# dusk-network/plonk

Measured on AMD Instinct MI355X. Metric: prove() wall-clock (ms) at 2^20 gates, lower is better.
Workload: dtype u32 limbs (Fr 256-bit / Fp 384-bit Montgomery)

## Files before the change

### __graft_entry__.py

```python
from __future__ import annotations

import concurrent.futures as cf
import os
import shutil
import subprocess
import sys

ROOT = os.path.dirname(os.path.abspath(__file__))
CSRC = os.path.join(ROOT, "plonk_amd", "csrc")
LIBDIR = os.path.join(ROOT, "plonk_amd", "lib")
OBJDIR = os.path.join(ROOT, "build", "obj")
LIB = os.path.join(LIBDIR, "libplonk_hip.so")
HIP_SOURCES = ["ntt.hip", "msm.hip", "msm_sort.hip", "capi.hip", "poly.hip", "prover.hip", "serial.hip", "comm.hip", "verify.hip", "diagnose.hip", "kzg.hip", "composer.hip", "msm_points.hip"]
MSM_LARGE_BITS = os.environ.get("PLONK_BUILD_MSM_LARGE_BITS", "19")
MSM_MEDIUM = os.environ.get("PLONK_BUILD_MSM_MEDIUM", "") == "1"
HIP_VARIANTS = [("msm.hip", "nbl" + MSM_LARGE_BITS, ["-DPLONK_MSM_NB_BITS=" + MSM_LARGE_BITS]),
                ("msm_sort.hip", "nbl" + MSM_LARGE_BITS, ["-DPLONK_MSM_NB_BITS=" + MSM_LARGE_BITS])]
if MSM_MEDIUM:
    HIP_VARIANTS += [("msm.hip", "nbm17", ["-DPLONK_MSM_NB_BITS=17", "-DPLONK_MSM_WITH_MEDIUM"]),
                     ("msm_sort.hip", "nbm17", ["-DPLONK_MSM_NB_BITS=17", "-DPLONK_MSM_WITH_MEDIUM"])]
    HIP_FLAGS_EXTRA = ["-DPLONK_MSM_WITH_MEDIUM"]
else:
    HIP_FLAGS_EXTRA = []
HIPCC = shutil.which("hipcc") or "/opt/rocm/bin/hipcc"
# ... 59 lines not shown
def build_dev_arith(verbose: bool = True) -> str:
    src = os.path.join(ROOT, "tests", "csrc", "dev_arith.hip")
    if not os.path.exists(src):
        return DEV_ARITH_LIB
    deps = [src, os.path.join(ROOT, "tests", "csrc", "arith_cases.hpp")] + _headers()
    if _newer(DEV_ARITH_LIB, deps):
        os.makedirs(os.path.dirname(DEV_ARITH_LIB), exist_ok=True)
        os.makedirs(OBJDIR, exist_ok=True)

        def compile_group(group: str) -> str:
            obj = os.path.join(OBJDIR, "dev_arith." + group + ".o")
            if _newer(obj, deps):
                subprocess.check_call([HIPCC, *HIP_FLAGS, "-DARITH_GROUP=ARITH_FAMILIES_" + group, "-c", src, "-o", obj])
            return obj

        with cf.ThreadPoolExecutor(max_workers=len(DEV_ARITH_GROUPS)) as ex:
            objs = list(ex.map(compile_group, DEV_ARITH_GROUPS))
        subprocess.check_call([HIPCC, "--offload-arch=gfx950", "-shared", "-fPIC", *objs, "-o", DEV_ARITH_LIB])
    if verbose:
        print(f"[build] {DEV_ARITH_LIB}")
    return DEV_ARITH_LIB


def build() -> None:
    with cf.ThreadPoolExecutor(max_workers=1) as side:
        dev_arith = side.submit(build_dev_arith)
        build_hip()
        build_oracle()
        build_fake_rccl()
        dev_arith.result()
    sys.path.insert(0, ROOT)
    import plonk_amd
    plonk_amd.load_library()


def smoke() -> None:
    sys.path.insert(0, ROOT)
    import random

    import plonk_amd
    from oracle import bls12_381 as E
    from oracle.fft import EvaluationDomain

    ctx = plonk_amd.Context(0)
    rnd = random.Random(7)
    L = 12
    coeffs = [rnd.randrange(E.Q) for _ in range((1 << 9) + 3)]
    got = ctx.ntt(coeffs, L, inverse=False, coset=True)
    assert got == EvaluationDomain(1 << L).coset_fft(coeffs), "NTT mismatch vs oracle"
    pts = [E.g1_mul(E.G1_GEN, rnd.randrange(1, E.Q)) for _ in range(64)]
# ... 9 lines not shown
```

### plonk_amd/csrc/poly.hip

```cpp
#include <cstdlib>

#include "plonk_internal.hpp"
#include "fr29.cuh"
#include "fp_safegcd.cuh"
#include "poly.hpp"

namespace plonk {

__device__ __forceinline__ Fr ldf(const Fr* p) {
  const uint4* q = reinterpret_cast<const uint4*>(p);
  uint4 a = q[0], b = q[1];
  Fr r;
  r.l[0] = a.x; r.l[1] = a.y; r.l[2] = a.z; r.l[3] = a.w;
  r.l[4] = b.x; r.l[5] = b.y; r.l[6] = b.z; r.l[7] = b.w;
  return r;
}
__device__ __forceinline__ void stf(Fr* p, const Fr& v) {
  uint4* q = reinterpret_cast<uint4*>(p);
  q[0] = make_uint4(v.l[0], v.l[1], v.l[2], v.l[3]);
  q[1] = make_uint4(v.l[4], v.l[5], v.l[6], v.l[7]);
}
__device__ __forceinline__ Fr small(uint32_t v, const Fr& one) {
  Fr acc = Fr::zero();
  Fr p = one;
  for (uint32_t b = v; b; b >>= 1) {
    if (b & 1) acc = acc + p;
    p = p.dbl();
  }
  return acc;
}

__global__ void fill_zero_kernel(Fr* p, uint64_t n) {
  const uint64_t i = (uint64_t)blockIdx.x * blockDim.x + threadIdx.x;
  if (i < n) stf(p + i, Fr::zero());
}

__global__ void blind_kernel(Fr* coeffs, uint64_t n, BlindArgs a) {
  const int i = threadIdx.x;
  if (i < a.count) {
    const Fr low = (uint64_t)i >= n ? a.b[i - n] : ldf(coeffs + i);
    stf(coeffs + i, low - a.b[i]);
    if (n + i >= (uint64_t)a.count) stf(coeffs + n + i, a.b[i]);
  }
}

__global__ void split_t_kernel(Fr* __restrict__ t, uint64_t n, uint64_t np, Fr* __restrict__ out, SplitArgs a) {
  const uint64_t i = (uint64_t)blockIdx.x * blockDim.x + threadIdx.x;
  const int part = blockIdx.y;
  if (i >= np) return;
  Fr v = Fr::zero();
  if (i < n) v = ldf(t + (uint64_t)part * n + i);
  else if (i == n) v = a.b[part];
  if (part >= 1 && i == 0) v = v - a.b[part - 1];
  stf(out + (uint64_t)part * np + i, v);
  if (part == 0 && i == n + 1) stf(t + 3 * n, ldf(t + 3 * n) - a.b[2]);
}

__global__ void __launch_bounds__(256) trimmed_len_kernel(const Fr* __restrict__ p, uint64_t n, unsigned long long* out) {
  __shared__ unsigned long long sh[256];
  const uint64_t i = (uint64_t)blockIdx.x * blockDim.x + threadIdx.x;
  unsigned long long v = 0;
  if (i < n && !ldf(p + i).is_zero()) v = i + 1;
  sh[threadIdx.x] = v;
  __syncthreads();
  for (int d = 128; d >= 1; d >>= 1) {
    if ((int)threadIdx.x < d) { const unsigned long long o = sh[threadIdx.x + d]; if (o > sh[threadIdx.x]) sh[threadIdx.x] = o; }
// ... 405 lines not shown
  }
  const uint64_t r = i - 1;
  Fr29 root = ld_slot(a.tw_lo29, r & ((1ull << a.lobits) - 1));
  if (a.use_hi) root = Fr29::mul(root, ld_slot(a.tw_hi29, r >> a.lobits));
  const Fr29 conv = tw29(k.conv), gamma_t = tw29(k.gamma_t), b32 = tw29(k.b32_t);
  Fr29 num, den;
#pragma unroll
  for (int j = 0; j < 4; ++j) {
    const Fr29 wg = Fr29::add_csub(Fr29::mul(ld29_(a.wires[j] + r), conv), gamma_t);
    const Fr29 nf = Fr29::add_csub(wg, Fr29::mul(root, tw29(k.bk_t[j])));
    const Fr29 df = Fr29::add_csub(wg, Fr29::mul(ld29_(a.sigma[j] + r), b32));
    num = j ? Fr29::mul(num, nf) : nf;
    den = j ? Fr29::mul(den, df) : df;
  }
  stf(a.num + i, num.to_fr());
  stf(a.den + i, den.to_fr());
}
__global__ void mul_arrays_kernel(Fr* __restrict__ a, const Fr* __restrict__ b, uint64_t n, int* zero_flag) {
  const uint64_t i = (uint64_t)blockIdx.x * blockDim.x + threadIdx.x;
  if (i >= n) return;
  const Fr y = ldf(b + i);
  if (zero_flag && y.is_zero()) *zero_flag = 1;
  stf(a + i, Fr29::mul(ld29_(a + i), Fr29::from_fr(y)).to_fr());
}

__device__ __forceinline__ Fr delta4(const Fr& f, const Fr& one) {
  const Fr two = one.dbl();
  return f * (f - one) * (f - two) * (f - two - one);
}

__device__ __forceinline__ Fr29 ld29(const Fr* p) { return Fr29::from_fr(ldf(p)); }
__device__ __forceinline__ Fr29 c29(const uint32_t (&v)[9]) {
  Fr29 r;
#pragma unroll
  for (int i = 0; i < 9; ++i) r.l[i] = v[i];
  return r;
}

struct WidgetConst {
  Tw conv, one_r, c1, c3, c9, c18, c81, c83, ed;
  Tw rg[4];
  Tw lg[5];
  Tw fx[4];
  Tw vr[3];
};
template <bool WIDGETS>
// ... 236 lines not shown
  if (first >= n) return;
  const Fr29 add = Fr29::from_fr(a.addend);
  const uint64_t e = first + exp_off;
  Fr29 p = tw29(a.one_t);
  bool started = false;
#pragma unroll 1
  for (uint32_t b = 0; b < a.nbits; ++b) {
    if ((e >> b) & 1) {
      const Fr29 w = tw29(a.pw[b]);
      p = started ? Fr29::mul(p, w) : w;
      started = true;
    }
  }
  const Fr29 step = tw29(a.pw[6]);
#pragma unroll 1
  for (int k = 0; k < E; ++k) {
    const uint64_t i = first + 64ull * k;
    if (i >= n) break;
    stf(dst + i, Fr29::mul(Fr29::add_csub(ld29_(src + i + src_off), add), p).to_fr());
    if (E > 1) p = Fr29::mul(p, step);
  }
}

__global__ void fold_kernel(const Fr* __restrict__ src, Fr* __restrict__ dst, uint64_t n, uint32_t extra, Fr c) {
  const uint64_t i = (uint64_t)blockIdx.x * blockDim.x + threadIdx.x;
  if (i >= n) return;
  Fr v = ldf(src + i);
  if (i < extra) v = v + c * ldf(src + n + i);
  stf(dst + i, v);
}

__global__ void shard_pack_kernel(ShardPackArgs a) {
  const uint64_t i = (uint64_t)blockIdx.x * blockDim.x + threadIdx.x;
  const uint32_t k = blockIdx.y, peer = blockIdx.z;
  if (i >= a.stride) return;
  const Fr* F = a.F[k];
  Fr v = Fr::zero();
  if (i < a.per) {
    const uint64_t idx = (uint64_t)peer * a.per + i;
    if (idx < a.n) v = ldf(F + idx);
  } else {
    v = ldf(F + (i - a.per));
  }
  stf(a.send + ((uint64_t)peer * a.cpr + k) * a.stride + i, v);
}

// ... 31 lines not shown
}

__global__ void shard_split_fix_kernel(ShardSplitFix a) {
  if (threadIdx.x != 0) return;
  auto own = [&](uint64_t idx) { return idx >= a.lo && idx < a.hi; };
  if (own(a.n)) { stf(a.parts[0] + a.n, a.b[0]); stf(a.parts[1] + a.n, a.b[1]); stf(a.parts[2] + a.n, a.b[2]); }
  if (own(0)) {
    stf(a.parts[1], ldf(a.parts[1]) - a.b[0]);
    stf(a.parts[2], ldf(a.parts[2]) - a.b[1]);
    stf(a.parts[3], ldf(a.parts[3]) - a.b[2]);
  }
}

static inline dim3 grid1(uint64_t n, int t) { return dim3((uint32_t)((n + t - 1) / t)); }

int poly_fill_zero(Ctx* c, Fr* p, uint64_t n) {
  if (!n) return PLONK_OK;
  hipLaunchKernelGGL(fill_zero_kernel, grid1(n, 256), dim3(256), 0, c->stream, p, n);
  HIP_TRY(hipGetLastError());
  return PLONK_OK;
}
int poly_blind(Ctx* c, Fr* coeffs, uint64_t n, const BlindArgs& a) {
  hipLaunchKernelGGL(blind_kernel, dim3(1), dim3(64), 0, c->stream, coeffs, n, a);
  HIP_TRY(hipGetLastError());
  return PLONK_OK;
}
int poly_split_t(Ctx* c, Fr* t, uint64_t n, uint64_t np, Fr* out, const SplitArgs& a) {
  hipLaunchKernelGGL(split_t_kernel, dim3((uint32_t)((np + 255) / 256), 3), dim3(256), 0, c->stream, t, n, np, out, a);
  HIP_TRY(hipGetLastError());
  return PLONK_OK;
}
int poly_trimmed_len(Ctx* c, const Fr* p, uint64_t n, unsigned long long* out_dev) {
  HIP_TRY(hipMemsetAsync(out_dev, 0, sizeof(unsigned long long), c->stream));
  hipLaunchKernelGGL(trimmed_len_kernel, grid1(n, 256), dim3(256), 0, c->stream, p, n, out_dev);
  HIP_TRY(hipGetLastError());
  return PLONK_OK;
}
int poly_sigma_evals(Ctx* c, const uint32_t* map_dev, const Fr* roots, Fr* out, uint64_t n, uint64_t stride, const SigmaArgs& a) {
  dim3 grid = grid1(n, 256);
  grid.y = 4;
  hipLaunchKernelGGL(sigma_evals_kernel, grid, dim3(256), 0, c->stream, map_dev, roots, out, n, stride, a);
  HIP_TRY(hipGetLastError());
  return PLONK_OK;
}
int poly_gather_wires(Ctx* c, const uint32_t* idx_dev, const Fr* values, Fr* wires, uint64_t constraints, uint64_t n) {
  dim3 grid = grid1(n, 256);
// ... 27 lines not shown
  else if (cfg == 2) BI_LAUNCH(64, 16);
  else if (cfg == 3) BI_LAUNCH(128, 8);
  else BI_LAUNCH(256, 16);
#undef BI_LAUNCH
  HIP_TRY(hipGetLastError());
  return PLONK_OK;
}
int poly_perm_terms(Ctx* c, const PermArgs& a) {
  PermConst k;
  k.conv = tw_of(Fr::from_u64(32));
  k.gamma_t = tw_of(a.gamma);
  for (int j = 0; j < 4; ++j) k.bk_t[j] = tw_of(a.beta * a.ks[j]);
  k.b32_t = tw_of(a.beta * Fr::from_u64(32));
  k.one_t = tw_of(Fr::one());
  PermArgs r = a;
  if (r.count == 0) { r.first = 0; r.count = a.n; }
  if (r.first + r.count > a.n) return (plonk::set_last_error("invalid argument", __func__, __FILE__, __LINE__), PLONK_ERR_ARG);
  hipLaunchKernelGGL(perm_terms_kernel, grid1(r.count, 128), dim3(128), 0, c->stream, r, k);
  HIP_TRY(hipGetLastError());
  return PLONK_OK;
}
int poly_mul_arrays(Ctx* c, Fr* a, const Fr* b, uint64_t n, int* zero_flag) {
  hipLaunchKernelGGL(mul_arrays_kernel, grid1(n, 256), dim3(256), 0, c->stream, a, b, n, zero_flag);
  HIP_TRY(hipGetLastError());
  return PLONK_OK;
}
int poly_quotient(Ctx* c, const QuotientArgs& q) {
  prof_begin(c, 3);
  WidgetConst wc{};
  if (q.has[QS_RANGE] | q.has[QS_LOGIC] | q.has[QS_FIXED] | q.has[QS_VAR]) {
    wc.conv = tw_of(Fr::from_u64(32));
    wc.one_r = tw_plain(Fr::one());
    wc.c1 = tw_of(Fr::one()); wc.c3 = tw_of(Fr::from_u64(3)); wc.c9 = tw_of(Fr::from_u64(9));
    wc.c18 = tw_of(Fr::from_u64(18)); wc.c81 = tw_of(Fr::from_u64(81)); wc.c83 = tw_of(Fr::from_u64(83));
    wc.ed = tw_of(q.edwards_d);
    Fr k = q.range_ch.sqr(), w = q.range_ch;
    for (int j = 0; j < 4; ++j) { wc.rg[j] = tw_of(w); w = w * k; }
    k = q.logic_ch.sqr();
    const Fr lk[5] = {k.sqr() * k, Fr::one(), k, k.sqr(), k.sqr().sqr()};
    for (int j = 0; j < 5; ++j) wc.lg[j] = tw_of(lk[j] * q.logic_ch);
    k = q.fixed_ch.sqr(); w = q.fixed_ch;
    for (int j = 0; j < 4; ++j) { wc.fx[j] = tw_of(w); w = w * k; }
    k = q.var_ch.sqr(); w = q.var_ch;
    for (int j = 0; j < 3; ++j) { wc.vr[j] = tw_of(w); w = w * k; }
    hipLaunchKernelGGL(quotient_kernel<true>, grid1(q.n8, 128), dim3(128), 0, c->stream, q, wc);
  } else {
// ... 106 lines not shown
  while (nbits < MP_BITS && (emax >> nbits)) ++nbits;
  Fr29 p = Fr29::twiddle_from_fr(x);
  for (uint32_t b = 0; b < nbits; ++b) {
    for (int i = 0; i < 9; ++i) a.pw[b].w[i] = p.l[i];
    p = Fr29::mul(p, p);
  }
  a.one_t = tw_of(Fr::one());
  a.addend = addend;
  a.nbits = nbits;
  a.zero_at = zero_at;
  if (n <= (1ull << 17)) hipLaunchKernelGGL(mul_powers_kernel<1>, grid1(n, 256), dim3(256), 0, c->stream, src, dst, n, a, src_off, exp_off);
  else if (n <= (1ull << 19)) hipLaunchKernelGGL(mul_powers_kernel<4>, grid1((n + 3) / 4 + 64, 256), dim3(256), 0, c->stream, src, dst, n, a, src_off, exp_off);
  else hipLaunchKernelGGL(mul_powers_kernel<16>, grid1((n + 15) / 16 + 64, 256), dim3(256), 0, c->stream, src, dst, n, a, src_off, exp_off);
}
int poly_ruffini(Ctx* c, const Fr* src, Fr* dst, uint64_t len, const Fr& z, const Fr& zinv, Fr* scratch, Fr* totals) {
  launch_mul_powers(c, src, scratch, len, z, 0, 0);
  int rc = scan_suffix_sum(c, scratch, len, totals);
  if (rc) return rc;
  launch_mul_powers(c, scratch, dst, len - 1, zinv, 1, 1, Fr::zero(), len - 1);
  HIP_TRY(hipGetLastError());
  return PLONK_OK;
}

__device__ __forceinline__ void st_slot(void* base, uint64_t idx, const Fr29& v) {
  uint32_t* w = reinterpret_cast<Fr29Slot*>(base)[idx].w;
#pragma unroll
  for (int i = 0; i < 9; ++i) w[i] = v.l[i];
  w[9] = 0; w[10] = 0; w[11] = 0;
}
__global__ void __launch_bounds__(256) kzg_powers_kernel(void* __restrict__ tab, uint32_t count, Tw xt, Tw one_t) {
  const uint32_t i = blockIdx.x * blockDim.x + threadIdx.x;
  if (i >= count) return;
  st_slot(tab, i, pow_tw(tw29(xt), i, tw29(one_t)));
}
__global__ void __launch_bounds__(256) power_array_kernel(Fr* __restrict__ out, uint64_t n, Tw xt, Tw one_t) {
  const uint64_t i = (uint64_t)blockIdx.x * blockDim.x + threadIdx.x;
  if (i >= n) return;
  stf(out + i, Fr29::mul(Fr29::from_fr(Fr::one()), pow_tw(tw29(xt), i, tw29(one_t))).to_fr());
}
__global__ void __launch_bounds__(256) kzg_trim_kernel(KzgDesc* __restrict__ desc) {
  __shared__ unsigned long long best;
  const Fr* p = desc[blockIdx.x].p;
  uint64_t hi = desc[blockIdx.x].len;
  while (hi) {
    if (!threadIdx.x) best = 0;
    __syncthreads();
// ... 141 lines not shown
```

### plonk_amd/csrc/poly.hpp

```cpp
#pragma once
#include "plonk_internal.hpp"

namespace plonk {

enum { QS_M = 0, QS_L, QS_R, QS_O, QS_F, QS_C, QS_ARITH, QS_RANGE, QS_LOGIC, QS_FIXED, QS_VAR, QS_COUNT };

struct BlindArgs {
  int count;
  Fr b[3];
};
struct SplitArgs {
  Fr b[3];
  uint64_t len4;
};
struct PermArgs {
  uint64_t n;
  uint64_t first = 0, count = 0;
  const Fr* wires[4];
  const Fr* sigma[4];
  Fr beta, gamma;
  Fr ks[4];
  const void* tw_lo29;
  const void* tw_hi29;
  uint32_t lobits;
// ... 91 lines not shown
  Fr* fold;
  Fr* partial;
  Fr point;
};
int poly_kzg_trim(Ctx* c, KzgDesc* desc_dev, uint32_t count);
int poly_kzg_powers(Ctx* c, void* vpow_dev, uint32_t count, const Fr& v);
int poly_power_array(Ctx* c, Fr* out, uint64_t n, const Fr& x);
int poly_kzg_fold_eval(Ctx* c, const KzgFoldArgs& a, Fr* evals_dev);
int poly_shift_down(Ctx* c, const Fr* src, Fr* dst, uint64_t len);

int poly_fold(Ctx* c, const Fr* src, Fr* dst, uint64_t n, uint32_t extra, const Fr& cn);
int poly_shard_pack(Ctx* c, const ShardPackArgs& a, uint32_t world);
int poly_shard_combine(Ctx* c, const ShardCombineArgs& a);
int poly_shard_split_fix(Ctx* c, const ShardSplitFix& a);
int poly_ruffini_local(Ctx* c, const Fr* src, uint64_t lo, uint64_t len, const Fr& z, Fr* scratch, Fr* totals);
int poly_ruffini_finish(Ctx* c, const Fr* scratch, Fr* dst, uint64_t lo, uint64_t len, const Fr& zinv, const Fr& carry, uint64_t last);

void prof_begin(Ctx* c, int slot);
void prof_end(Ctx* c, int slot);
void prof_host_add(Ctx* c, int slot, double ms);

int poly_fill_zero(Ctx* c, Fr* p, uint64_t n);
int poly_blind(Ctx* c, Fr* coeffs, uint64_t n, const BlindArgs& a);
int poly_split_t(Ctx* c, Fr* t, uint64_t n, uint64_t np, Fr* out, const SplitArgs& a);
int poly_trimmed_len(Ctx* c, const Fr* p, uint64_t n, unsigned long long* out_dev);
int poly_scatter_pi(Ctx* c, Fr* dense, const uint64_t* idx, const Fr* val, uint64_t count);
int poly_sigma_evals(Ctx* c, const uint32_t* map_dev, const Fr* roots, Fr* out, uint64_t n, uint64_t stride, const SigmaArgs& a);
int poly_gather_wires(Ctx* c, const uint32_t* idx_dev, const Fr* values, Fr* wires, uint64_t constraints, uint64_t n);
int poly_batch_inverse(Ctx* c, Fr* v, uint64_t n, bool twiddle_form = false);
int poly_perm_terms(Ctx* c, const PermArgs& a);
int poly_mul_arrays(Ctx* c, Fr* a, const Fr* b, uint64_t n, int* zero_flag);
int poly_quotient(Ctx* c, const QuotientArgs& q);
int poly_dealias(Ctx* c, Fr* t, uint64_t nq, const Fr low[7], const Fr& g_inv);
int poly_l1(Ctx* c, const Fr* linear, Fr* l1, uint64_t n8, const L1Args& a);
int poly_scale_array(Ctx* c, Fr* v, uint64_t n, const Fr& s);
int poly_from_mont(Ctx* c, const Fr* src, Fr* dst, uint64_t n);
void quotient_const(const Fr& c, int shift, uint32_t out[9]);
void quotient_data(const Fr& c, uint32_t out[9]);
int poly_eval(Ctx* c, EvalArgs& a, int count, uint64_t max_len, Fr* out_dev);
int poly_lincomb(Ctx* c, const LinCombArgs& a);
int poly_ruffini(Ctx* c, const Fr* src, Fr* dst, uint64_t len, const Fr& z, const Fr& zinv, Fr* scratch, Fr* totals);
int scan_prefix_product(Ctx* c, Fr* data, uint64_t n, Fr* totals);
uint32_t scan_prefix_blocks(uint64_t n);
int scan_prefix_product_local(Ctx* c, Fr* data, uint64_t n, Fr* totals);
int scan_prefix_product_apply(Ctx* c, Fr* data, uint64_t n, const Fr* totals, const Fr& carry_twiddle);
int scan_suffix_sum(Ctx* c, Fr* data, uint64_t n, Fr* totals);

}
```

### plonk_amd/csrc/prover.hip

```cpp
#include <cstdlib>
#include <cstring>
#include <random>
#include <string>
#include <vector>

#include "poly.hpp"
#include "transcript.hpp"
#include <chrono>

#include "hostg1.hpp"
#include "finish_pool.hpp"
#include "widgets.hpp"
#include "permutation.hpp"
#include "diagnose.hpp"
#include "composer.hpp"

static_assert(plonk::DQ_M == plonk::QS_M && plonk::DQ_ARITH == plonk::QS_ARITH && plonk::DQ_VAR == plonk::QS_VAR &&
              plonk::DQ_COUNT == plonk::QS_COUNT, "diagnose_core.hpp selector ids");
static_assert(plonk::WQS_RANGE == plonk::QS_RANGE && plonk::WQS_LOGIC == plonk::QS_LOGIC && plonk::WQS_FIXED == plonk::QS_FIXED &&
              plonk::WQS_VAR == plonk::QS_VAR && plonk::WQS_COUNT == plonk::QS_COUNT, "widgets.hpp selector ids");

namespace plonk {

struct Prover {
// ... 724 lines not shown
  const uint64_t n = p->n, n8 = p->n8, np = p->np;
  const uint32_t L = p->logn;
  NttTables* tbn;
  PTRY(ntt_tables(c, L, false, &tbn));
  const Fr omega = omega_of(L);

  Transcript tr((const uint8_t*)p->label.data(), p->label.size());
  seed_transcript(tr, p, pi_val, pi_count);

  uint8_t comm[11][48];
  HostGap gap{c};
  GapScope gap_scope(&gap);
  const bool lag = p->lag_on;
  auto wire_polynomials = [&](Fr* ntt_tmp, int k0 = 0, int k1 = 4) -> int {
    prof_begin(c, 4);
    for (int k = k0; k < k1; ++k) {
      Fr* wp = p->wpoly + k * np;
      if (p->wires_pending) HIP_TRY(hipStreamWaitEvent(c->stream, p->ev_wire[k], 0));
      PTRY(ntt_device(c, wires_dev + k * n, wp, ntt_tmp, L, true, false, n));
      BlindArgs ba;
      ba.count = 2;
      ba.b[0] = bl[2 * k];
      ba.b[1] = bl[2 * k + 1];
      PTRY(poly_fill_zero(c, wp + n, np - n));
      PTRY(poly_blind(c, wp, n, ba));
    }
    prof_end(c, 4);
    for (int k = k0; k < k1; ++k)
      HIP_TRY(hipMemcpyAsync(p->low_host + 7 * k, p->wpoly + k * np, 7 * sizeof(Fr), hipMemcpyDeviceToHost, c->stream));
    return PLONK_OK;
  };
  const int bc_cfg = c->cfg.wire_by_column;
  const bool by_column = lag && p->wires_pending && p->world == 1 && bc_cfg >= 0 && (L > 18 || bc_cfg > 0);
  const bool polys_on_side = lag && !by_column && (c->cfg.wire_polys_side >= 0 ? c->cfg.wire_polys_side == 1 : L <= 19);
  if (!polys_on_side && !by_column) PTRY(wire_polynomials(p->tmp8));
  if (lag && by_column) {
    HIP_TRY(hipMemcpyAsync(p->wscal, bl, 8 * sizeof(Fr), hipMemcpyHostToDevice, c->stream));
  } else if (lag) {
    for (int k = 0; k < 4; ++k)
      if (p->wires_pending) HIP_TRY(hipStreamWaitEvent(c->stream, p->ev_wire[k], 0));
    HIP_TRY(hipMemcpyAsync(p->wscal, bl, 8 * sizeof(Fr), hipMemcpyHostToDevice, c->stream));
  }
  SideJoin side_join{c};
  uint64_t pi_len = 0;
  const int side_defer_env = c->cfg.side_defer;
  const bool defer_size = L <= 18 || (L == 19 && !by_column);
  const bool side_defer = side_defer_env >= 0 ? side_defer_env >= 1 : defer_size;
  const bool side_defer_z = side_defer_env >= 0 ? side_defer_env == 1 : defer_size;
// ... 53 lines not shown
    SideScopeAfter side(c, p->ev_acc);
    PTRY(side_round1());
  }
  PTRY(fetch_commitments(p, 0, 4, comm));
  tr.append_commitment("a_comm", comm[0]);
  tr.append_commitment("b_comm", comm[1]);
  tr.append_commitment("c_comm", comm[2]);
  tr.append_commitment("d_comm", comm[3]);

  const Fr beta = tr.challenge_scalar("beta");
  tr.append_scalar("beta", beta);
  const Fr gamma = tr.challenge_scalar("gamma");
  {
    prof_begin(c, 4);
    PermArgs pa;
    pa.n = n;
    for (int k = 0; k < 4; ++k) { pa.wires[k] = wires_dev + k * n; pa.sigma[k] = p->sigma_n + k * n; }
    pa.beta = beta; pa.gamma = gamma;
    pa.ks[0] = Fr::one(); pa.ks[1] = fr_small(7); pa.ks[2] = fr_small(13); pa.ks[3] = fr_small(17);
    pa.tw_lo29 = tbn->tw_lo29; pa.tw_hi29 = tbn->tw_hi29; pa.lobits = L < 13 ? L : 13; pa.use_hi = L > 13;
    pa.num = p->scratch; pa.den = p->scratch + np;
    gap.launching();
    HIP_TRY(hipMemsetAsync(p->flag_dev, 0, sizeof(int), c->stream));
    PTRY(poly_perm_terms(c, pa));
    PTRY(poly_batch_inverse(c, pa.den, n, true));
    PTRY(poly_mul_arrays(c, pa.num, pa.den, n, p->flag_dev));
    PTRY(scan_prefix_product(c, pa.num, n, p->totals));
    if (!z_from_evals) {
      PTRY(ntt_device(c, pa.num, p->zpoly, p->tmp8, L, true, false, n));
      BlindArgs ba;
      ba.count = 3;
      ba.b[0] = bl[8]; ba.b[1] = bl[9]; ba.b[2] = bl[10];
      PTRY(poly_fill_zero(c, p->zpoly + n, np - n));
      PTRY(poly_blind(c, p->zpoly, n, ba));
    }
    prof_end(c, 4);
  }
  auto z_polynomial = [&](Fr* ntt_tmp) -> int {
    PTRY(ntt_device(c, p->scratch, p->zpoly, ntt_tmp, L, true, false, n));
    BlindArgs ba;
    ba.count = 3;
    ba.b[0] = bl[8]; ba.b[1] = bl[9]; ba.b[2] = bl[10];
    PTRY(poly_fill_zero(c, p->zpoly + n, np - n));
    PTRY(poly_blind(c, p->zpoly, n, ba));
    return PLONK_OK;
  };
  if (z_from_evals) {
    HIP_TRY(hipMemcpyAsync(p->wscal + 8, bl + 8, 3 * sizeof(Fr), hipMemcpyHostToDevice, c->stream));
    if (!side_defer_z) {
      SideScope side(c, p->ev_ready);
      PTRY(z_polynomial(p->tmp8b));
      HIP_TRY(hipMemcpyAsync(p->low_host + 28, p->zpoly, 7 * sizeof(Fr), hipMemcpyDeviceToHost, c->stream));
      HIP_TRY(hipEventRecord(p->ev_zlow, c->stream));
      PTRY(ntt_device(c, p->zpoly, p->cos, p->tmp8b, L + p->lq, false, true, n + 3));
      HIP_TRY(hipEventRecord(p->ev_side, c->side_stream));
    }
    {
      AccMark mark(c, side_defer_z ? p->ev_acc : nullptr);
      const Fr* sc[1] = {p->scratch};
      const Fr* tl[1] = {p->wscal + 8};
      const uint64_t ms[1] = {n + 3}, sp[1] = {n};
      PTRY(msm_group(p, sc, ms, 1, 4, p->lag_table, p->lag_n, tl, sp));
    }
    if (side_defer_z) {
      SideScopeAfter side(c, p->ev_acc);
      PTRY(z_polynomial(p->tmp8b));
      HIP_TRY(hipMemcpyAsync(p->low_host + 28, p->zpoly, 7 * sizeof(Fr), hipMemcpyDeviceToHost, c->stream));
// ... 143 lines not shown
  Fr inv_z, inv_zm1;
  {
    const Fr zm1 = z_ch - one;
    const Fr a = z_zero ? one : z_ch, b = zm1.is_zero() ? one : zm1;
    const Fr iab = fr_inv_gcd(a * b);
    inv_z = iab * b;
    inv_zm1 = iab * a;
  }
  if (z_zero || zw.is_zero()) return PLONK_ERR_STATE;
  const Fr v_w = tr.challenge_scalar("v_w_challenge");
  {
    gap.launching();
    SideScope side(c, p->ev_ready);
    LinCombArgs la;
    la.t[0].p = p->zpoly; la.t[0].len = n + 3; la.t[0].s = one;
    la.t[1].p = p->wpoly; la.t[1].len = n + 2; la.t[1].s = v_w;
    la.t[2].p = p->wpoly + np; la.t[2].len = n + 2; la.t[2].s = v_w.sqr();
    la.t[3].p = p->wpoly + 3 * np; la.t[3].len = n + 2; la.t[3].s = v_w.sqr() * v_w;
    la.count = 4;
    la.len = np - 1;
    la.constant = Fr::zero();
    la.out = p->tmp8;
    PTRY(poly_lincomb(c, la));
    PTRY(poly_ruffini(c, p->tmp8, p->wit2, np - 1, zw, inv_z * p->omega_inv, p->scratch + np, p->totals + 8192));
    HIP_TRY(hipEventRecord(p->ev_side, c->side_stream));
  }
  const Fr pi_eval = public_input_eval(p, pi_idx, pi_val, pi_count, z_ch, zh);
  const Fr bz = beta * z_ch;
  const Fr lin_a = (ev.a + bz + gamma) * (ev.b + fr_small(7) * bz + gamma) * (ev.c + fr_small(13) * bz + gamma) *
                   (ev.d + fr_small(17) * bz + gamma) * alpha;
  const Fr lin_b = (ev.a + beta * ev.s1 + gamma) * (ev.b + beta * ev.s2 + gamma) * (ev.c + beta * ev.s3 + gamma) *
                   (beta * ev.z) * alpha;
  Fr l1_z;
  if (z_n == one) l1_z = (z_ch == one) ? one : Fr::zero();
  else l1_z = zh * n_inv * inv_zm1;
  const Fr c_range = range_identity(range_ch, ev) * range_ch;
  const Fr c_logic = logic_identity(logic_ch, ev) * logic_ch;
  const Fr c_fixed = fixed_identity(fixed_ch, ev, edwards_d) * fixed_ch;
  const Fr c_var = var_identity(var_ch, ev, edwards_d) * var_ch;
  const Fr nzh = zh.neg();
  Fr vp[12];
  vp[0] = one;
  for (int k = 1; k < 12; ++k) vp[k] = vp[k - 1] * v;
  {
    LinCombArgs la;
    int k = 0;
    const Fr* P = p->polys;
// ... 9 lines not shown
    term(P + P_QLOGIC * np, p->poly_len[P_QLOGIC], c_logic);
    term(P + P_QFIXED * np, p->poly_len[P_QFIXED], c_fixed);
    term(P + P_QVAR * np, p->poly_len[P_QVAR], c_var);
    term(P + P_S1 * np, p->poly_len[P_S1], vp[5]);
    term(P + P_S2 * np, p->poly_len[P_S2], vp[6]);
    term(P + P_S3 * np, p->poly_len[P_S3], vp[7]);
    term(P + P_S4 * np, p->poly_len[P_S4], lin_b.neg());
    term(p->zpoly, n + 3, lin_a + l1_z * alpha.sqr());
    term(p->wpoly, n + 2, vp[1]);
    term(p->wpoly + np, n + 2, vp[2]);
    term(p->wpoly + 2 * np, n + 2, vp[3]);
    term(p->wpoly + 3 * np, n + 2, vp[4]);
    term(p->tparts, n + 1, nzh);
    term(p->tparts + np, n + 1, nzh * z_n);
    term(p->tparts + 2 * np, n + 1, nzh * z_n.sqr());
    term(t4, t4_len, nzh * z_n.sqr() * z_n);
    la.count = k;
    la.len = np - 1;
    la.constant = pi_eval;
    la.out = p->agg;
    gap.launching();
    PTRY(poly_lincomb(c, la));
  }
  PTRY(poly_ruffini(c, p->agg, p->wit, np - 1, z_ch, inv_z, p->scratch, p->totals));
  HIP_TRY(hipMemcpyAsync(p->evout + 15, p->scratch, sizeof(Fr), hipMemcpyDeviceToDevice, c->stream));
  HIP_TRY(hipMemcpyAsync(p->ev_host + 15, p->evout + 15, sizeof(Fr), hipMemcpyDeviceToHost, c->stream));
  HIP_TRY(hipStreamWaitEvent(c->main_stream, p->ev_side, 0));
  {
    const Fr* sc[2] = {p->wit, p->wit2};
    const uint64_t ms[2] = {np - 2, np - 2};
    PTRY(msm_group(p, sc, ms, 2, 9));
  }
  PTRY(fetch_commitments(p, 9, 2, comm + 9));
  if (!quotient_identity_holds(p->ev_host[15], ev, alpha, beta, gamma, l1_z, vp)) return PLONK_ERR_UNSAT;

  write_proof(proof, comm, ev);
  return PLONK_OK;
}

static int prover_prove_sharded(Prover* p, const Fr* wires_dev, const uint64_t* pi_idx, const Fr* pi_val, uint64_t pi_count,
                                const Fr* bl, uint8_t proof[1008]) {
  Ctx* c = p->c;
  if (p->srs_gen != c->srs_gen) return (set_last_error("prover is bound to an SRS that was replaced on its context", __func__, __FILE__, __LINE__), PLONK_ERR_STATE);
  const uint64_t n = p->n, np = p->np, qn = p->qn;
  const uint32_t L = p->logn, W = (uint32_t)p->world, cpr = p->cpr, Q = p->Q;
  const uint64_t lo = p->lo, hi = p->hi;
  NttTables* tbn;
// ... 1020 lines not shown
```

Measured before the change: 32.05.

## Fuse permutation grand product, Ruffini division and blinding tail into fewer kernels

Replaces the four-kernel permutation pipeline (terms, batch inverse, multiply, prefix product) with a single-pass grand product. It computes numerator prefix and denominator suffix products per block and does one field inversion in a totals kernel, so the separate batch inversion is avoided. Ruffini division is rewritten as a fused block-scan plus apply over powers of z taken from a small power table. The zero-fill and blinding launches are merged into one kernel. The aim is to cut kernel launches and memory passes over the 2^20-element arrays, at the cost of extra multiplications per element and a single-threaded serial zero-fill loop over the blinding tail.

```diff
diff --git a/__graft_entry__.py b/__graft_entry__.py
--- a/__graft_entry__.py
+++ b/__graft_entry__.py
@@ -105,10 +105,27 @@
     return DEV_ARITH_LIB
 
 
+DEV_POLY_CHAINS_LIB = os.path.join(ROOT, "tests", "_build", "libdev_poly_chains.so")
+
+
+def build_dev_poly_chains(verbose: bool = True) -> str:
+    src = os.path.join(ROOT, "tests", "csrc", "dev_poly_chains.hip")
+    if not os.path.exists(src):
+        return DEV_POLY_CHAINS_LIB
+    if _newer(DEV_POLY_CHAINS_LIB, [src, LIB] + _headers()):
+        os.makedirs(os.path.dirname(DEV_POLY_CHAINS_LIB), exist_ok=True)
+        subprocess.check_call([HIPCC, *HIP_FLAGS, "-shared", src, "-o", DEV_POLY_CHAINS_LIB, "-L" + LIBDIR, "-lplonk_hip",
+                               "-Wl,-rpath,$ORIGIN/../../plonk_amd/lib"])
+    if verbose:
+        print(f"[build] {DEV_POLY_CHAINS_LIB}")
+    return DEV_POLY_CHAINS_LIB
+
+
 def build() -> None:
     with cf.ThreadPoolExecutor(max_workers=1) as side:
         dev_arith = side.submit(build_dev_arith)
         build_hip()
+        build_dev_poly_chains()
         build_oracle()
         build_fake_rccl()
         dev_arith.result()
diff --git a/plonk_amd/csrc/poly.hip b/plonk_amd/csrc/poly.hip
--- a/plonk_amd/csrc/poly.hip
+++ b/plonk_amd/csrc/poly.hip
@@ -42,6 +42,16 @@
     stf(coeffs + i, low - a.b[i]);
     if (n + i >= (uint64_t)a.count) stf(coeffs + n + i, a.b[i]);
   }
+}
+
+__global__ void __launch_bounds__(64) blind_tail_kernel(Fr* coeffs, uint64_t n, uint64_t np, BlindArgs a) {
+  const int i = threadIdx.x;
+  if (i < a.count) {
+    const Fr low = (uint64_t)i >= n ? a.b[i - n] : ldf(coeffs + i);
+    stf(coeffs + i, low - a.b[i]);
+    if (n + i >= (uint64_t)a.count) stf(coeffs + n + i, a.b[i]);
+  }
+  for (uint64_t j = n + a.count + i; j < np; j += 64) stf(coeffs + j, Fr::zero());
 }
 
 __global__ void split_t_kernel(Fr* __restrict__ t, uint64_t n, uint64_t np, Fr* __restrict__ out, SplitArgs a) {
@@ -493,6 +503,127 @@
   const Fr y = ldf(b + i);
   if (zero_flag && y.is_zero()) *zero_flag = 1;
   stf(a + i, Fr29::mul(ld29_(a + i), Fr29::from_fr(y)).to_fr());
+}
+
+template <int E>
+__global__ void __launch_bounds__(SCAN_T) gp_local_kernel(PermArgs a, PermConst k, Fr* __restrict__ totals, uint32_t nb, int* zero_flag) {
+  __shared__ uint32_t shp[9][SCAN_T], shs[9][SCAN_T];
+  const int t = threadIdx.x;
+  const uint64_t base = (uint64_t)blockIdx.x * (SCAN_T * E) + (uint64_t)t * E;
+  const Fr29 one_t = tw29(k.one_t), conv = tw29(k.conv), gamma_t = tw29(k.gamma_t), b32 = tw29(k.b32_t);
+  Fr29 pn[E], d[E];
+  Fr29 acc = one_t;
+#pragma unroll
+  for (int e = 0; e < E; ++e) {
+    const uint64_t i = base + e;
+    Fr29 num = one_t, den = one_t;
+    if (i > 0 && i < a.n) {
+      const uint64_t r = i - 1;
+      Fr29 root = ld_slot(a.tw_lo29, r & ((1ull << a.lobits) - 1));
+      if (a.use_hi) root = Fr29::mul(root, ld_slot(a.tw_hi29, r >> a.lobits));
+#pragma unroll
+      for (int j = 0; j < 4; ++j) {
+        const Fr29 wg = Fr29::add_csub(Fr29::mul(ld29_(a.wires[j] + r), conv), gamma_t);
+        const Fr29 nf = Fr29::add_csub(wg, Fr29::mul(root, tw29(k.bk_t[j])));
+        const Fr29 df = Fr29::add_csub(wg, Fr29::mul(ld29_(a.sigma[j] + r), b32));
+        num = j ? Fr29::mul(num, nf) : nf;
+        den = j ? Fr29::mul(den, df) : df;
+      }
+      if (den.to_fr().is_zero()) {
+        *zero_flag = 1;
+        num = Fr29::zero();
+        den = one_t;
+      }
+    }
+    acc = Fr29::mul(acc, num);
+    pn[e] = acc;
+    d[e] = den;
+  }
+  Fr29 sd = d[E - 1];
+#pragma unroll
+  for (int e = E - 2; e >= 0; --e) {
+    pn[e] = Fr29::mul(pn[e], sd);
+    sd = Fr29::mul(sd, d[e]);
+  }
+  Fr29 pfx = acc, sfx = sd;
+  for (int s = 1; s < SCAN_T; s <<= 1) {
+    ps_put(shp, t, pfx);
+    ps_put(shs, t, sfx);
+    __syncthreads();
+    if (t >= s) pfx = Fr29::mul(pfx, ps_get(shp, t - s));
+    if (t + s < SCAN_T) sfx = Fr29::mul(sfx, ps_get(shs, t + s));
+    __syncthreads();
+  }
+  ps_put(shp, t, pfx);
+  ps_put(shs, t, sfx);
+  __syncthreads();
+  if (t == SCAN_T - 1) stf(totals + blockIdx.x, pfx.to_fr());
+  if (t == 0) stf(totals + nb + blockIdx.x, sfx.to_fr());
+  Fr29 outer = t ? ps_get(shp, t - 1) : one_t;
+  if (t + 1 < SCAN_T) outer = Fr29::mul(outer, ps_get(shs, t + 1));
+#pragma unroll
+  for (int e = 0; e < E; ++e)
+    if (base + e < a.n) stf(a.num + base + e, Fr29::mul(pn[e], outer).to_fr());
+}
+__global__ void __launch_bounds__(SCAN_T) gp_totals_kernel(Fr* __restrict__ totals, uint32_t nb, uint32_t per, PScanArgs a) {
+  __shared__ uint32_t shp[9][SCAN_T], shs[9][SCAN_T], shinv[9];
+  const int t = threadIdx.x;
+  const Fr29 one_t = tw29(a.one_t);
+  Fr* tn = totals;
+  const Fr* td = totals + nb;
+  Fr29 pfx = one_t, sfx = one_t;
+  for (uint32_t k = 0; k < per; ++k) {
+    const uint32_t i = t * per + k;
+    if (i < nb) {
+      pfx = Fr29::mul(pfx, ld29_(tn + i));
+      sfx = Fr29::mul(sfx, ld29_(td + i));
+    }
+  }
+  for (int s = 1; s < SCAN_T; s <<= 1) {
+    ps_put(shp, t, pfx);
+    ps_put(shs, t, sfx);
+    __syncthreads();
+    if (t >= s) pfx = Fr29::mul(pfx, ps_get(shp, t - s));
+    if (t + s < SCAN_T) sfx = Fr29::mul(sfx, ps_get(shs, t + s));
+    __syncthreads();
+  }
+  ps_put(shp, t, pfx);
+  ps_put(shs, t, sfx);
+  __syncthreads();
+  if (t == 0) {
+    const Fr29 r = Fr29::mul(fr29_inv_gcd_tw(sfx), tw29(a.one_r));
+#pragma unroll
+    for (int i = 0; i < 9; ++i) shinv[i] = r.l[i];
+  }
+  __syncthreads();
+  Fr29 cn;
+#pragma unroll
+  for (int i = 0; i < 9; ++i) cn.l[i] = shinv[i];
+  if (t) cn = Fr29::mul(cn, ps_get(shp, t - 1));
+  for (uint32_t k = 0; k < per; ++k) {
+    const uint32_t i = t * per + k;
+    if (i < nb) {
+      const Fr29 x = ld29_(tn + i);
+      stf(tn + i, cn.to_fr());
+      cn = Fr29::mul(cn, x);
+    }
+  }
+  Fr29 cd = t + 1 < SCAN_T ? ps_get(shs, t + 1) : one_t;
+  for (uint32_t k = per; k-- > 0;) {
+    const uint32_t i = t * per + k;
+    if (i < nb) {
+      stf(tn + i, Fr29::mul(ld29_(tn + i), cd).to_fr());
+      cd = Fr29::mul(cd, ld29_(td + i));
+    }
+  }
+}
+template <int E>
+__global__ void __launch_bounds__(SCAN_T) gp_apply_kernel(Fr* __restrict__ data, uint64_t n, const Fr* __restrict__ carries) {
+  const Fr29 off = ld29_(carries + blockIdx.x);
+  const uint64_t base = (uint64_t)blockIdx.x * (SCAN_T * E) + (uint64_t)threadIdx.x * E;
+#pragma unroll
+  for (int e = 0; e < E; ++e)
+    if (base + e < n) stf(data + base + e, Fr29::mul(ld29_(data + base + e), off).to_fr());
 }
 
 __device__ __forceinline__ Fr delta4(const Fr& f, const Fr& one) {
@@ -775,6 +906,88 @@
   }
 }
 
+struct PowTab {
+  Tw pw[MP_BITS];
+  Tw one_t;
+  uint32_t nbits;
+};
+__device__ __forceinline__ Fr29 pow_tab(const PowTab& a, uint64_t e) {
+  Fr29 p = tw29(a.one_t);
+  bool started = false;
+#pragma unroll 1
+  for (uint32_t b = 0; b < a.nbits; ++b) {
+    if ((e >> b) & 1) {
+      const Fr29 w = tw29(a.pw[b]);
+      p = started ? Fr29::mul(p, w) : w;
+      started = true;
+    }
+  }
+  return p;
+}
+__global__ void __launch_bounds__(SCAN_T) ruffini_block_kernel(const Fr* __restrict__ src, Fr* __restrict__ scratch, uint64_t n,
+                                                               Fr* __restrict__ totals, PowTab a) {
+  __shared__ Fr sh[SCAN_T];
+  const int t = threadIdx.x;
+  const uint64_t base = (uint64_t)blockIdx.x * SCAN_BLOCK + (uint64_t)t * SCAN_E;
+  const int cnt = base >= n ? 0 : (n - base < (uint64_t)SCAN_E ? (int)(n - base) : SCAN_E);
+  Fr v[SCAN_E];
+  if (cnt) {
+    const uint64_t g0 = n - base - cnt;
+    Fr29 p = pow_tab(a, g0);
+    const Fr29 x = tw29(a.pw[0]);
+#pragma unroll
+    for (int k = SCAN_E - 1; k >= 0; --k) {
+      if (k < cnt) {
+        v[k] = Fr29::mul(ld29_(src + (n - 1 - (base + k))), p).to_fr();
+        if (k) p = Fr29::mul(p, x);
+      }
+    }
+  }
+  Fr acc = Fr::zero();
+#pragma unroll
+  for (int k = 0; k < SCAN_E; ++k) {
+    if (k < cnt) acc = acc + v[k];
+    v[k] = acc;
+  }
+  sh[t] = acc;
+  __syncthreads();
+  for (int d = 1; d < SCAN_T; d <<= 1) {
+    Fr y = Fr::zero();
+    const bool take = t >= d;
+    if (take) y = sh[t - d];
+    __syncthreads();
+    if (take) sh[t] = y + sh[t];
+    __syncthreads();
+  }
+  const Fr excl = t ? sh[t - 1] : Fr::zero();
+  if (t == SCAN_T - 1) stf(totals + blockIdx.x, sh[t]);
+#pragma unroll
+  for (int k = 0; k < SCAN_E; ++k)
+    if (k < cnt) stf(scratch + (n - 1 - (base + k)), excl + v[k]);
+}
+__global__ void __launch_bounds__(SCAN_T) ruffini_apply_kernel(Fr* __restrict__ scratch, Fr* __restrict__ dst, uint64_t n,
+                                                               const Fr* __restrict__ totals, PowTab a) {
+  const int t = threadIdx.x;
+  if (blockIdx.x == 0 && t == 0) stf(dst + n - 1, Fr::zero());
+  const uint64_t base = (uint64_t)blockIdx.x * SCAN_BLOCK + (uint64_t)t * SCAN_E;
+  const int cnt = base >= n ? 0 : (n - base < (uint64_t)SCAN_E ? (int)(n - base) : SCAN_E);
+  if (!cnt) return;
+  const Fr off = blockIdx.x ? ldf(totals + blockIdx.x - 1) : Fr::zero();
+  const uint64_t g0 = n - base - cnt;
+  Fr29 p = pow_tab(a, g0);
+  const Fr29 x = tw29(a.pw[0]);
+#pragma unroll
+  for (int k = SCAN_E - 1; k >= 0; --k) {
+    if (k < cnt) {
+      const uint64_t gi = n - 1 - (base + k);
+      const Fr s = off + ldf(scratch + gi);
+      if (gi == 0) stf(scratch, s);
+      else stf(dst + gi - 1, Fr29::mul(Fr29::from_fr(s), p).to_fr());
+      if (k) p = Fr29::mul(p, x);
+    }
+  }
+}
+
 __global__ void fold_kernel(const Fr* __restrict__ src, Fr* __restrict__ dst, uint64_t n, uint32_t extra, Fr c) {
   const uint64_t i = (uint64_t)blockIdx.x * blockDim.x + threadIdx.x;
   if (i >= n) return;
@@ -852,6 +1065,12 @@
 }
 int poly_blind(Ctx* c, Fr* coeffs, uint64_t n, const BlindArgs& a) {
   hipLaunchKernelGGL(blind_kernel, dim3(1), dim3(64), 0, c->stream, coeffs, n, a);
+  HIP_TRY(hipGetLastError());
+  return PLONK_OK;
+}
+int poly_blind_tail(Ctx* c, Fr* coeffs, uint64_t n, uint64_t np, const BlindArgs& a) {
+  if (np < n + (uint64_t)a.count) return (plonk::set_last_error("invalid argument", __func__, __FILE__, __LINE__), PLONK_ERR_ARG);
+  hipLaunchKernelGGL(blind_tail_kernel, dim3(1), dim3(64), 0, c->stream, coeffs, n, np, a);
   HIP_TRY(hipGetLastError());
   return PLONK_OK;
 }
@@ -925,6 +1144,33 @@
 }
 int poly_mul_arrays(Ctx* c, Fr* a, const Fr* b, uint64_t n, int* zero_flag) {
   hipLaunchKernelGGL(mul_arrays_kernel, grid1(n, 256), dim3(256), 0, c->stream, a, b, n, zero_flag);
+  HIP_TRY(hipGetLastError());
+  return PLONK_OK;
+}
+uint32_t grand_product_blocks(uint64_t n, int geometry) {
+  const uint64_t blk = (uint64_t)SCAN_T * (geometry ? geometry : pscan_e(n));
+  return (uint32_t)((n + blk - 1) / blk);
+}
+int poly_grand_product(Ctx* c, const PermArgs& a, int* zero_flag, int geometry) {
+  if (geometry != 0 && geometry != 2 && geometry != 8) return (plonk::set_last_error("invalid argument", __func__, __FILE__, __LINE__), PLONK_ERR_ARG);
+  const int e = geometry ? geometry : pscan_e(a.n);
+  const uint32_t nb = grand_product_blocks(a.n, e);
+  if (!a.n || nb > SCAN_T * SCAN_MAXPER || !zero_flag) return (plonk::set_last_error("invalid argument", __func__, __FILE__, __LINE__), PLONK_ERR_ARG);
+  PermConst k;
+  k.conv = tw_of(Fr::from_u64(32));
+  k.gamma_t = tw_of(a.gamma);
+  for (int j = 0; j < 4; ++j) k.bk_t[j] = tw_of(a.beta * a.ks[j]);
+  k.b32_t = tw_of(a.beta * Fr::from_u64(32));
+  k.one_t = tw_of(Fr::one());
+  PScanArgs s{};
+  s.one_t = k.one_t;
+  s.one_r = tw_plain(Fr::one());
+  Fr* totals = a.den;
+  if (e == 2) hipLaunchKernelGGL(gp_local_kernel<2>, dim3(nb), dim3(SCAN_T), 0, c->stream, a, k, totals, nb, zero_flag);
+  else hipLaunchKernelGGL(gp_local_kernel<8>, dim3(nb), dim3(SCAN_T), 0, c->stream, a, k, totals, nb, zero_flag);
+  hipLaunchKernelGGL(gp_totals_kernel, dim3(1), dim3(SCAN_T), 0, c->stream, totals, nb, (nb + SCAN_T - 1) / SCAN_T, s);
+  if (e == 2) hipLaunchKernelGGL(gp_apply_kernel<2>, dim3(nb), dim3(SCAN_T), 0, c->stream, a.num, a.n, totals);
+  else hipLaunchKernelGGL(gp_apply_kernel<8>, dim3(nb), dim3(SCAN_T), 0, c->stream, a.num, a.n, totals);
   HIP_TRY(hipGetLastError());
   return PLONK_OK;
 }
@@ -1077,6 +1323,31 @@
   return PLONK_OK;
 }
 
+static PowTab pow_tab_of(const Fr& x, uint64_t emax) {
+  PowTab a;
+  uint32_t nbits = 1;
+  while (nbits < MP_BITS && (emax >> nbits)) ++nbits;
+  Fr29 p = Fr29::twiddle_from_fr(x);
+  for (uint32_t b = 0; b < nbits; ++b) {
+    for (int i = 0; i < 9; ++i) a.pw[b].w[i] = p.l[i];
+    p = Fr29::mul(p, p);
+  }
+  for (uint32_t b = nbits; b < MP_BITS; ++b) a.pw[b] = a.pw[0];
+  a.one_t = tw_of(Fr::one());
+  a.nbits = nbits;
+  return a;
+}
+int poly_ruffini_fused(Ctx* c, const Fr* src, Fr* dst, uint64_t len, const Fr& z, const Fr& zinv, Fr* scratch, Fr* totals) {
+  if (!len) return PLONK_OK;
+  const uint32_t nb = (uint32_t)((len + SCAN_BLOCK - 1) / SCAN_BLOCK);
+  if (nb > SCAN_T * SCAN_MAXPER) return (plonk::set_last_error("invalid argument", __func__, __FILE__, __LINE__), PLONK_ERR_ARG);
+  hipLaunchKernelGGL(ruffini_block_kernel, dim3(nb), dim3(SCAN_T), 0, c->stream, src, scratch, len, totals, pow_tab_of(z, len - 1));
+  if (nb > 1) hipLaunchKernelGGL(scan_totals_kernel<false>, dim3(1), dim3(SCAN_T), 0, c->stream, totals, nb, (nb + SCAN_T - 1) / SCAN_T);
+  hipLaunchKernelGGL(ruffini_apply_kernel, dim3(nb), dim3(SCAN_T), 0, c->stream, scratch, dst, len, (const Fr*)totals, pow_tab_of(zinv, len - 1));
+  HIP_TRY(hipGetLastError());
+  return PLONK_OK;
+}
+
 __device__ __forceinline__ void st_slot(void* base, uint64_t idx, const Fr29& v) {
   uint32_t* w = reinterpret_cast<Fr29Slot*>(base)[idx].w;
 #pragma unroll
diff --git a/plonk_amd/csrc/poly.hpp b/plonk_amd/csrc/poly.hpp
--- a/plonk_amd/csrc/poly.hpp
+++ b/plonk_amd/csrc/poly.hpp
@@ -137,6 +137,7 @@
 
 int poly_fill_zero(Ctx* c, Fr* p, uint64_t n);
 int poly_blind(Ctx* c, Fr* coeffs, uint64_t n, const BlindArgs& a);
+int poly_blind_tail(Ctx* c, Fr* coeffs, uint64_t n, uint64_t np, const BlindArgs& a);
 int poly_split_t(Ctx* c, Fr* t, uint64_t n, uint64_t np, Fr* out, const SplitArgs& a);
 int poly_trimmed_len(Ctx* c, const Fr* p, uint64_t n, unsigned long long* out_dev);
 int poly_scatter_pi(Ctx* c, Fr* dense, const uint64_t* idx, const Fr* val, uint64_t count);
@@ -145,6 +146,8 @@
 int poly_batch_inverse(Ctx* c, Fr* v, uint64_t n, bool twiddle_form = false);
 int poly_perm_terms(Ctx* c, const PermArgs& a);
 int poly_mul_arrays(Ctx* c, Fr* a, const Fr* b, uint64_t n, int* zero_flag);
+uint32_t grand_product_blocks(uint64_t n, int geometry = 0);
+int poly_grand_product(Ctx* c, const PermArgs& a, int* zero_flag, int geometry = 0);
 int poly_quotient(Ctx* c, const QuotientArgs& q);
 int poly_dealias(Ctx* c, Fr* t, uint64_t nq, const Fr low[7], const Fr& g_inv);
 int poly_l1(Ctx* c, const Fr* linear, Fr* l1, uint64_t n8, const L1Args& a);
@@ -155,6 +158,7 @@
 int poly_eval(Ctx* c, EvalArgs& a, int count, uint64_t max_len, Fr* out_dev);
 int poly_lincomb(Ctx* c, const LinCombArgs& a);
 int poly_ruffini(Ctx* c, const Fr* src, Fr* dst, uint64_t len, const Fr& z, const Fr& zinv, Fr* scratch, Fr* totals);
+int poly_ruffini_fused(Ctx* c, const Fr* src, Fr* dst, uint64_t len, const Fr& z, const Fr& zinv, Fr* scratch, Fr* totals);
 int scan_prefix_product(Ctx* c, Fr* data, uint64_t n, Fr* totals);
 uint32_t scan_prefix_blocks(uint64_t n);
 int scan_prefix_product_local(Ctx* c, Fr* data, uint64_t n, Fr* totals);
diff --git a/plonk_amd/csrc/prover.hip b/plonk_amd/csrc/prover.hip
--- a/plonk_amd/csrc/prover.hip
+++ b/plonk_amd/csrc/prover.hip
@@ -770,8 +770,7 @@
       ba.count = 2;
       ba.b[0] = bl[2 * k];
       ba.b[1] = bl[2 * k + 1];
-      PTRY(poly_fill_zero(c, wp + n, np - n));
-      PTRY(poly_blind(c, wp, n, ba));
+      PTRY(poly_blind_tail(c, wp, n, np, ba));
     }
     prof_end(c, 4);
     for (int k = k0; k < k1; ++k)
@@ -871,17 +870,13 @@
     pa.num = p->scratch; pa.den = p->scratch + np;
     gap.launching();
     HIP_TRY(hipMemsetAsync(p->flag_dev, 0, sizeof(int), c->stream));
-    PTRY(poly_perm_terms(c, pa));
-    PTRY(poly_batch_inverse(c, pa.den, n, true));
-    PTRY(poly_mul_arrays(c, pa.num, pa.den, n, p->flag_dev));
-    PTRY(scan_prefix_product(c, pa.num, n, p->totals));
+    PTRY(poly_grand_product(c, pa, p->flag_dev));
     if (!z_from_evals) {
       PTRY(ntt_device(c, pa.num, p->zpoly, p->tmp8, L, true, false, n));
       BlindArgs ba;
       ba.count = 3;
       ba.b[0] = bl[8]; ba.b[1] = bl[9]; ba.b[2] = bl[10];
-      PTRY(poly_fill_zero(c, p->zpoly + n, np - n));
-      PTRY(poly_blind(c, p->zpoly, n, ba));
+      PTRY(poly_blind_tail(c, p->zpoly, n, np, ba));
     }
     prof_end(c, 4);
   }
@@ -890,8 +885,7 @@
     BlindArgs ba;
     ba.count = 3;
     ba.b[0] = bl[8]; ba.b[1] = bl[9]; ba.b[2] = bl[10];
-    PTRY(poly_fill_zero(c, p->zpoly + n, np - n));
-    PTRY(poly_blind(c, p->zpoly, n, ba));
+    PTRY(poly_blind_tail(c, p->zpoly, n, np, ba));
     return PLONK_OK;
   };
   if (z_from_evals) {
@@ -1081,7 +1075,7 @@
     la.constant = Fr::zero();
     la.out = p->tmp8;
     PTRY(poly_lincomb(c, la));
-    PTRY(poly_ruffini(c, p->tmp8, p->wit2, np - 1, zw, inv_z * p->omega_inv, p->scratch + np, p->totals + 8192));
+    PTRY(poly_ruffini_fused(c, p->tmp8, p->wit2, np - 1, zw, inv_z * p->omega_inv, p->scratch + np, p->totals + 8192));
     HIP_TRY(hipEventRecord(p->ev_side, c->side_stream));
   }
   const Fr pi_eval = public_input_eval(p, pi_idx, pi_val, pi_count, z_ch, zh);
@@ -1137,7 +1131,7 @@
     gap.launching();
     PTRY(poly_lincomb(c, la));
   }
-  PTRY(poly_ruffini(c, p->agg, p->wit, np - 1, z_ch, inv_z, p->scratch, p->totals));
+  PTRY(poly_ruffini_fused(c, p->agg, p->wit, np - 1, z_ch, inv_z, p->scratch, p->totals));
   HIP_TRY(hipMemcpyAsync(p->evout + 15, p->scratch, sizeof(Fr), hipMemcpyDeviceToDevice, c->stream));
   HIP_TRY(hipMemcpyAsync(p->ev_host + 15, p->evout + 15, sizeof(Fr), hipMemcpyDeviceToHost, c->stream));
   HIP_TRY(hipStreamWaitEvent(c->main_stream, p->ev_side, 0));
```

Result: no change. 31.85, median of 4 (-0.6%).
